# thowell/DirectTrajectoryOptimization.jl

Measured on AMD Instinct MI355X. Metric: SQP iterations/sec + Jacobian nnz/sec, acrobot T=1000, 1->8 GPU, higher is better.
Workload: dtype f64; 1 GPU; acrobot swing-up, implicit midpoint h=0.05, T=1000, exact Hessians, 524288 independent instances per GPU (BASELINE.json configs[2]); horizon=1000, instances_per_gpu=524288, instances_total=524288, num_variables=4999, num_constraint=4004, jacobian_nnz=25982, hessian_key=40971, parallelism=instance sharding x1

## Files before the change

directtrajectoryoptimization.jl_amd/csrc/dto_solver.cpp:

```cpp
#include <hip/hip_runtime.h>

#include <algorithm>
#include <chrono>
#include <cmath>
#include <cstdio>
#include <cstdint>
#include <cstdlib>
#include <cstring>
#include <vector>

#include "../../include/dto.h"
#include "dto_kkt_kernels.hpp"
#include "dto_im_kernels.hpp"
#include "dto_wide_kernels.hpp"
#include "dto_border_kernels.hpp"
#include "dto_problem.hpp"
#include "dto_host_globalization.hpp"

#define HIP_TRY(expr)                                       \
  do {                                                      \
    hipError_t e_ = (expr);                                 \
    if (e_ != hipSuccess) return dto::hip_fail(e_, #expr);  \
  } while (0)

namespace dto {


struct SolverBufs {
  DevBuf<double> wtile;
  DevBuf<int> d_inst_of_slot, d_src_slot;
  DevBuf<double> repack_tmp;
  DevBuf<double> sigx, sigc;
  DevBuf<int> d_ioff;
  DevBuf<int64_t> d_recoff, d_facoff;
  DevBuf<dto_stage_run> d_runs;
  DevBuf<double> d_lo, d_hi;
  DevBuf<double> z, lam, zl, zu, s, zs;
  DevBuf<int> tile_fwd_tag, tile_bwd_tag, fwd_started;
  DevBuf<double> qn;
  DevBuf<double> refq, refvz, refvl, rec_bak;
  DevBuf<double> z_alt, lam_alt;
  DevBuf<double> dz, dlam, ds;
  DevBuf<double> rec, fac, part, lspart, scal, filt;
  DevBuf<double> csum, sfac, xsep, cacc, cpart;
  DevBuf<int> csync;
  DevBuf<int> d_cstart_all;
};

struct SolverState : SolverBufs {
  int64_t B = 0;
  int G = 0;
  int64_t Ni = 0, rec_total = 0, fac_total = 0, n_bnd = 0;
  bool use_wtile = false;
  int G_active = 0;
  std::vector<int> inst_of_slot, slot_of_inst;
  bool use_sigx = false, use_sigc = false, assembled = false;
  std::vector<int> ioff;
  std::vector<int64_t> recoff, facoff;
  int n_runs = 0;
  int sweep_tag = 0;
  hipStream_t stream_lo = nullptr;
  hipEvent_t ev_fork = nullptr, ev_join = nullptr;
  SolverState* cols = nullptr;
  int fuse_state = 0;
  int sb = 8;
  int P = 1;
  int P0 = 1;
  int P_cap = 1;
  int forced_P = 0;
  int n_simd = 1024;
  std::vector<int> cstart;
  int* d_cstart = nullptr;
  dto_kkt_info info{};
  dto_solver_opts opt{};
  dto_options user{};
  bool begun = false;
  std::vector<double> h_scal;

  void release() {
    static_cast<SolverBufs&>(*this) = SolverBufs();
    d_cstart = nullptr; n_runs = 0; fuse_state = 0; sweep_tag = 0;
    if (stream_lo) { (void)hipStreamDestroy(stream_lo); stream_lo = nullptr; }
    if (ev_fork) { (void)hipEventDestroy(ev_fork); ev_fork = nullptr; }
    if (ev_join) { (void)hipEventDestroy(ev_join); ev_join = nullptr; }
    use_wtile = false;
    use_sigx = use_sigc = assembled = false;
    G_active = 0;
    inst_of_slot.clear(); slot_of_inst.clear();
    B = 0; G = 0;
    delete cols; cols = nullptr;
  }
  ~SolverState() { release(); }
};
template <class S>
struct ReleaseOnError {
  S* s;
  ~ReleaseOnError() { if (s) s->release(); }
};

struct ImBufs {
  DevBuf<int> d_aoff, d_doff, d_coff, d_boff, d_ioff;
  DevBuf<double> d_lo, d_hi;
  DevBuf<double> A, R, D, C, Bd;
  DevBuf<double> part, lspart, scal, filt, wbuf;
  DevBuf<int> phase;
  DevBuf<int> lists;
  DevBuf<int> ctr;
};
struct ImState : ImBufs {
  int64_t B = 0;
  dto_im_info info{};
  std::vector<int> aoff, doff, coff, boff, ioff;
  int64_t a_total = 0, d_total = 0, c_total = 0, b_total = 0, Ni = 0, n_bnd = 0;
  bool use_w = false;
  int* h_ctr = nullptr;
  int nwin_e = 1, nwin_l = 1;
  dto_solver_opts opt{};
  dto_options user{};
  bool begun = false;
  int iter_base = 0;
  int64_t passes = 0;
  std::vector<double> h_scal;

  void release() {
    static_cast<ImBufs&>(*this) = ImBufs();
    if (h_ctr) (void)hipHostFree(h_ctr);
    h_ctr = nullptr;
    B = 0; begun = false; use_w = false;
  }
  ~ImState() { release(); }
};

static void default_opts(dto_solver_opts& o, const dto_options& u) {
  o.tol = u.tol; o.s_max = u.s_max; o.dual_inf_tol = u.dual_inf_tol; o.constr_viol_tol = u.constr_viol_tol;
  o.compl_inf_tol = u.compl_inf_tol; o.max_iter = u.max_iter;
  o.acceptable_tol = u.acceptable_tol; o.acceptable_iter = u.acceptable_iter; o.acceptable_dual_inf_tol = u.acceptable_dual_inf_tol;
  o.acceptable_constr_viol_tol = u.acceptable_constr_viol_tol; o.acceptable_compl_inf_tol = u.acceptable_compl_inf_tol;
  o.acceptable_obj_change_tol = u.acceptable_obj_change_tol;
  o.diverging_iterates_tol = u.diverging_iterates_tol; o.mu_target = u.mu_target;
  o.mu_init = u.mu_init; o.kappa_eps = 10.0; o.kappa_mu = 0.2; o.theta_mu = 1.5; o.tau_min = 0.99;
  o.bound_push = 1e-2; o.bound_frac = 1e-2;
  o.delta_c = u.delta_c; o.delta_w_init = u.delta_w_init; o.delta_w_min = 1e-20; o.delta_w_max = 1e20;
  if (const char* e = getenv("DTO_DW_FLOOR")) { const double v = atof(e); if (v > 0.0) o.delta_w_min = v; }
  o.kappa_w_minus = 1.0 / 3.0; o.kappa_w_plus = 8.0; o.kappa_w_plus_first = 100.0;
  o.delta_w_exact_cap = 100.0;
  if (const char* e = getenv("DTO_EXACT_CAP")) o.delta_w_exact_cap = atof(e);
  o.eta_armijo = 1e-4; o.rho_penalty = 0.1; o.piv_tol = 1e-9;
  o.max_refactor = 9;
  o.watchdog_trigger = 2; o.watchdog_trials = 4;
  if (const char* e = getenv("DTO_WATCHDOG")) sscanf(e, "%d,%d", &o.watchdog_trigger, &o.watchdog_trials);
  o.newton_only = 0; o.fixed_delta_w = 0.0;
  o.warm = 0; o.mu_warm = 0.0;
  o.ls_penalty = u.line_search == DTO_LS_PENALTY_FILTER ? 1 : 0; o.ls_switch = u.penalty_switch_theta;
  if (const char* e = getenv("DTO_LS_MERIT")) o.ls_penalty = atoi(e);
  o.pen_gn = 1;
  o.qn_lbfgs = u.hessian_approximation == DTO_HESSIAN_LBFGS ? 1 : 0;
  o.cost_hess_scale = o.qn_lbfgs ? 0.0 : 1.0;
  if (const char* e = getenv("DTO_PEN_GN")) o.pen_gn = atoi(e);
}

struct BorderStats;

static int bordered_step(Problem* p, const dto_batch* b, const double* mu, int64_t ldmu, const double* dw, double delta_c,
                         double* dx, int64_t lddx, double* dmu, int64_t lddmu, int* ok_out, BorderStats* stats, bool pin_fixed = false,
                         const double* gdiag = nullptr, const double* gshift = nullptr);
static int general_solve_batch(Problem* p, const dto_options* opt, const dto_batch* b, double* x_out, int64_t ldxo,
                               double* mu_out, int64_t ldmuo, int32_t* status, int32_t* iterations);

struct WideKkt {
  int64_t B = 0;
  bool assembled = false, factored = false, own_params = false, use_sigx = false, use_sigc = false;
  double delta_w = 0.0, delta_c = 0.0;
  DevBuf<double> z, mu, params, sigx, sigc;
  DevBuf<int> flags;
  DevBuf<double> ws;
  DevBuf<double> ref_r, ref_d;
};
struct KktBorder {
  bool valid = false;
  int nb = 0;
  int64_t B = 0;
  DevBuf<double> g, y;
  DevBuf<double> part;
  DevBuf<double> lu, yw;
  DevBuf<double> v0;
  DevBuf<int> iw;
};
static inline void kkt_border_taken(Problem* p) {
  if (p->kkt_border) p->kkt_border->valid = false;
}
static inline void wide_fac_taken(Problem* p) {
  if (p->wide_kkt) p->wide_kkt->factored = false;
  kkt_border_taken(p);
}
static inline void wide_args_no_linear(dto_wide_args& a) {
  a.sigma_x = a.sigma_c = nullptr; a.ldsx = a.ldsc = 0; a.nneg = nullptr;
  a.rhs_x = a.rhs_c = nullptr; a.ldrx = a.ldrc = 0;
  a.nrhs = a.rhs0 = 0; a.ws = nullptr;
  a.kmul_s = 0;
}

static int wide_step(Problem* p, const dto_batch* b, const double* mu, int64_t ldmu, double delta_w, double delta_c,
                     double* dx, int64_t lddx, double* dmu, int64_t lddmu, int* inertia_ok) {
  int rc = p->ensure_device();
  if (rc) return rc;
  dto_wide_info info;
  p->vt->wide_info(&info);
  const Layout& L = p->L;
  if (L.Nstage != 0 || L.Ngen != 0) return set_error(DTO_ERR_UNSUPPORTED, "wide-stage models: dynamics rows and bounds only");
  hipStream_t st = (hipStream_t)b->stream;
  wide_fac_taken(p);
  const size_t need = (size_t)b->B * (size_t)L.T * (size_t)info.fac_stage;
  HIP_TRY(p->wide_fac.grow(need));
  HIP_TRY(p->wide_flags.grow((size_t)b->B));
  dto_wide_args a;
  a.T = L.T; a.B = b->B;
  a.kind = p->d_kind; a.zoff = p->d_zoff; a.woff = p->d_woff; a.cdoff = p->d_cdoff;
  a.params = b->params ? b->params : p->d_params; a.ldw = b->params ? b->ldp : 0;
  a.z = b->x; a.ldz = b->ldx; a.mu = mu; a.ldmu = ldmu;
  a.delta_w = delta_w; a.delta_c = delta_c; a.piv_tol = 1e-9;
  a.dz = dx; a.lddz = lddx; a.dmu = dmu; a.lddmu = lddmu;
  a.fac = p->wide_fac; a.flags = p->wide_flags; a.Nc = L.Nc;
  a.fixed_lo = a.fixed_hi = nullptr; a.ldb = 0; a.dw_inst = nullptr; a.gam_inst = nullptr; a.active = nullptr; a.stats = nullptr; a.merit = nullptr;
  a.zl = a.zu = nullptr; a.mu_inst = nullptr; a.tau_min = 0.99;
  wide_args_no_linear(a);
  a.prof = nullptr;
  if (const char* e = getenv("DTO_WIDE_PROF")) a.prof = (long long*)(uintptr_t)strtoull(e, nullptr, 0);
  const int lrc = p->vt->launch_wide(DTO_WIDE_STEP, &a, (void*)st);
  if (lrc != 0) return hip_fail((hipError_t)lrc, "wide kernel launch");
  if (inertia_ok) {
    std::vector<int> fl((size_t)b->B);
    HIP_TRY(hipMemcpyAsync(fl.data(), p->wide_flags, fl.size() * sizeof(int), hipMemcpyDeviceToHost, st));
    HIP_TRY(hipStreamSynchronize(st));
    *inertia_ok = 1;
    for (int v : fl) if (!v) *inertia_ok = 0;
  }
  return DTO_OK;
// ... 882 lines not shown
  for (int t = 0; t < L.T; ++t) {
    const int k = L.kind[t];
    S.ioff[t + 1] = S.ioff[t] + S.info.n_ineq[k];
    S.recoff[t + 1] = S.recoff[t] + S.info.rec_size[k];
    S.facoff[t + 1] = S.facoff[t] + (seq_only ? S.info.fac_size_seq[k] : S.info.fac_size[k]);
  }
  S.Ni = S.ioff[L.T]; S.rec_total = S.recoff[L.T]; S.fac_total = S.facoff[L.T];
  for (int64_t rows : {(int64_t)L.Nz, (int64_t)L.Nc, (int64_t)L.Nw, (int64_t)S.Ni, S.rec_total, S.fac_total})
    if (rows >= (int64_t)1 << 22)
      return set_error(DTO_ERR_UNSUPPORTED, "problem too large for the solver path: an array of one instance exceeds 4194303 rows");
  S.n_bnd = S.Ni;
  for (int64_t i = 0; i < L.Nz; ++i) {
    if (L.var_lo[i] == L.var_hi[i]) continue;
    if (std::isfinite(L.var_lo[i])) ++S.n_bnd;
    if (std::isfinite(L.var_hi[i])) ++S.n_bnd;
  }
  {
    std::vector<dto_stage_run> runs;
    auto bounded = [&](int t) {
      for (int i = L.zoff[t]; i < L.zoff[t] + L.nx[t] + L.nu[t]; ++i)
        if (L.var_lo[i] == L.var_hi[i] || std::isfinite(L.var_lo[i]) || std::isfinite(L.var_hi[i])) return 1;
      return 0;
    };
    auto zstep = [&](int t) { return t + 1 < L.T ? L.zoff[t + 1] - L.zoff[t] : L.nx[t] + L.nu[t]; };
    for (int t = 0; t < L.T;) {
      dto_stage_run r{};
      r.kind = L.kind[t]; r.t0 = t; r.bounded = bounded(t);
      r.z0 = L.zoff[t]; r.cd0 = L.cdoff[t]; r.cc0 = L.ccoff[t]; r.io0 = S.ioff[t]; r.w0 = L.woff[t];
      r.rec0 = S.recoff[t]; r.fac0 = S.facoff[t];
      r.zs = zstep(t);
      int e = t + 1;
      if (e < L.T && L.kind[e] == r.kind && bounded(e) == r.bounded && zstep(e) == r.zs && L.zoff[e] - L.zoff[t] == r.zs) {
        r.cds = L.cdoff[e] - L.cdoff[t]; r.ccs = L.ccoff[e] - L.ccoff[t]; r.ios = S.ioff[e] - S.ioff[t]; r.ws = L.woff[e] - L.woff[t];
        r.recs = S.recoff[e] - S.recoff[t]; r.facs = S.facoff[e] - S.facoff[t];
        for (;; ++e) {
          if (e >= L.T || L.kind[e] != r.kind || bounded(e) != r.bounded || zstep(e) != r.zs) break;
          const int64_t n = e - t;
          if (L.zoff[e] != r.z0 + n * r.zs || L.cdoff[e] != r.cd0 + n * r.cds || L.ccoff[e] != r.cc0 + n * r.ccs ||
              S.ioff[e] != r.io0 + n * r.ios || L.woff[e] != r.w0 + n * r.ws || S.recoff[e] != r.rec0 + n * r.recs ||
              S.facoff[e] != r.fac0 + n * r.facs)
            break;
        }
      }
      r.t1 = e;
      runs.push_back(r);
      t = e;
    }
    S.n_runs = (int)runs.size();
    HIP_TRY(S.d_runs.alloc(runs.size()));
    HIP_TRY(hipMemcpy(S.d_runs, runs.data(), runs.size() * sizeof(dto_stage_run), hipMemcpyHostToDevice));
  }
  const size_t lanes = (size_t)S.G * 64;
  HIP_TRY(S.d_ioff.alloc(L.T + 1));
  HIP_TRY(hipMemcpy(S.d_ioff, S.ioff.data(), (L.T + 1) * sizeof(int), hipMemcpyHostToDevice));
  HIP_TRY(S.d_recoff.alloc(L.T + 1));
  HIP_TRY(hipMemcpy(S.d_recoff, S.recoff.data(), (L.T + 1) * sizeof(int64_t), hipMemcpyHostToDevice));
  HIP_TRY(S.d_facoff.alloc(L.T + 1));
  HIP_TRY(hipMemcpy(S.d_facoff, S.facoff.data(), (L.T + 1) * sizeof(int64_t), hipMemcpyHostToDevice));
  HIP_TRY(S.d_lo.alloc(L.Nz));
  HIP_TRY(S.d_hi.alloc(L.Nz));
  HIP_TRY(hipMemcpy(S.d_lo, L.var_lo.data(), L.Nz * sizeof(double), hipMemcpyHostToDevice));
  HIP_TRY(hipMemcpy(S.d_hi, L.var_hi.data(), L.Nz * sizeof(double), hipMemcpyHostToDevice));
  HIP_TRY(S.z.alloc_zeroed(lanes * L.Nz));
  HIP_TRY(S.lam.alloc_zeroed(lanes * L.Nc));
  if (S.n_bnd > S.Ni) {
    HIP_TRY(S.zl.alloc_zeroed(lanes * L.Nz));
    HIP_TRY(S.zu.alloc_zeroed(lanes * L.Nz));
  }
  HIP_TRY(S.s.alloc_zeroed(lanes * S.Ni));
  HIP_TRY(S.zs.alloc_zeroed(lanes * S.Ni));
  HIP_TRY(S.dz.alloc_zeroed(lanes * L.Nz));
  HIP_TRY(S.dlam.alloc_zeroed(lanes * L.Nc));
  HIP_TRY(S.ds.alloc_zeroed(lanes * S.Ni));
  HIP_TRY(S.rec.alloc_zeroed(lanes * S.rec_total));
  HIP_TRY(S.fac.alloc_zeroed(lanes * S.fac_total));
  {
    const int64_t want = ((int64_t)S.G * L.T) / 1024;
    S.sb = (int)std::max<int64_t>(1, std::min<int64_t>(DTO_SB, want));
    if (const char* e = getenv("DTO_STAGE_BLOCK")) S.sb = std::max(1, std::min((int)DTO_SB, atoi(e)));
  }
  const size_t nblk = ((size_t)L.T + S.sb - 1) / S.sb;
  HIP_TRY(S.part.alloc_zeroed(lanes * nblk * S.info.npart));
  HIP_TRY(S.lspart.alloc_zeroed(lanes * nblk * 2 * S.info.ls_trials));
  HIP_TRY(S.scal.alloc_zeroed(lanes * S.info.nscal));
  HIP_TRY(S.tile_fwd_tag.alloc_zeroed((size_t)S.G + 8));
  HIP_TRY(S.tile_bwd_tag.alloc_zeroed((size_t)S.G + 8));
  HIP_TRY(S.fwd_started.alloc_zeroed(16));
  HIP_TRY(S.filt.alloc_zeroed(lanes * 2 * S.info.filter_cap));
  {
    const int q_lo = (S.P_cap > S.P) ? 1 : S.P, q_hi = S.P_cap;
    std::vector<int> all;
    int off_cur = 0;
    for (int q = q_lo; q <= q_hi; ++q) {
      if (q == S.P) off_cur = (int)all.size();
      for (int c = 0; c <= q; ++c) all.push_back((int)(((int64_t)c * L.T) / q));
    }
    S.cstart.assign(all.begin() + off_cur, all.begin() + off_cur + S.P + 1);
    HIP_TRY(S.d_cstart_all.alloc(all.size()));
    HIP_TRY(hipMemcpy(S.d_cstart_all, all.data(), all.size() * sizeof(int), hipMemcpyHostToDevice));
    S.d_cstart = S.d_cstart_all + off_cur;
  }
  HIP_TRY(S.csum.alloc_zeroed(lanes * (size_t)S.P_cap * S.info.chunk_sum_size));
  HIP_TRY(S.sfac.alloc_zeroed(lanes * (size_t)S.P_cap * S.info.sep_fac_size));
  HIP_TRY(S.xsep.alloc_zeroed(lanes * (size_t)S.P_cap * S.info.nx));
  HIP_TRY(S.cacc.alloc_zeroed(lanes * (size_t)S.P_cap * 4));
  HIP_TRY(S.cpart.alloc_zeroed(lanes * (size_t)S.P_cap * 16));
  HIP_TRY(S.csync.alloc_zeroed((size_t)S.G * 4));
  S.h_scal.assign(lanes * S.info.nscal, 0.0);
  HIP_TRY(hipDeviceSynchronize());
  guard.s = nullptr;
  return DTO_OK;
}

static void fill_kkt_args(Problem* p, dto_kkt_args& a) {
  SolverState& S = *p->solver;
  const Layout& L = p->L;
  std::memset(&a, 0, sizeof(a));
  a.T = L.T; a.B = S.B; a.G = S.G;
  a.Nz = L.Nz; a.Nc = L.Nc - L.Ngen; a.Ni = S.Ni;
  a.n_mult = L.Nc; a.n_bnd = S.n_bnd;
  a.kind = p->d_kind; a.zoff = p->d_zoff; a.woff = p->d_woff; a.cdoff = p->d_cdoff; a.ccoff = p->d_ccoff;
  a.ioff = S.d_ioff; a.recoff = S.d_recoff; a.facoff = S.d_facoff;
  a.rec_total = S.rec_total; a.fac_total = S.fac_total;
  a.runs = S.d_runs; a.n_runs = S.n_runs;
  a.lo = S.d_lo; a.hi = S.d_hi; a.params = p->d_params;
  a.wtile = S.use_wtile ? S.wtile : nullptr; a.Nw = L.Nw;
  a.sigx = (S.opt.newton_only && S.use_sigx) ? S.sigx : nullptr;
  a.sigc = (S.opt.newton_only && S.use_sigc) ? S.sigc : nullptr;
  a.z_next = nullptr; a.lam_next = nullptr;
  a.tile_fwd_tag = a.tile_bwd_tag = nullptr; a.sweep_tag = 0; a.fwd_started = nullptr;
  a.z = S.z; a.lam = S.lam; a.zl = S.zl; a.zu = S.zu; a.s = S.s; a.zs = S.zs;
  a.dz = S.dz; a.dlam = S.dlam; a.ds = S.ds;
  a.rec = S.rec; a.fac = S.fac; a.part = S.part; a.lspart = S.lspart; a.scal = S.scal; a.filt = S.filt;
  a.inst_of_slot = S.d_inst_of_slot;
  a.fwd_rounds = fwd_rounds_per_launch();
  a.qn = S.qn; a.qn_mode = 0; a.qn_col = 0;
  a.refq = S.refq; a.refvz = S.refvz; a.refvl = S.refvl;
  a.prof = nullptr;
  if (const char* e = getenv("DTO_KKT_PROF")) a.prof = (long long*)(uintptr_t)strtoull(e, nullptr, 0);
  a.P = S.P; a.cstart = S.d_cstart; a.csum = S.csum; a.sfac = S.sfac; a.xsep = S.xsep; a.cacc = S.cacc; a.cpart = S.cpart;
  a.sb = S.sb;
  {
    const char* e = getenv("DTO_FUSE_JOIN");
    const char* mt = getenv("DTO_FUSE_JOIN_TILES");
    const int max_tiles = mt ? atoi(mt) : 2;
    a.csync = ((!e || atoi(e) != 0) && (S.G_active > 0 ? S.G_active : S.G) <= max_tiles) ? S.csync : nullptr;
  }
  {
    const char* e = getenv("DTO_SEP_CR");
    const bool cr_on = !e || atoi(e) != 0;
    a.sep_cr = !cr_on ? 0 : (S.B <= DTO_SEP_CR_MAX_INST ? 1 : (S.P >= 16 ? 2 : 0));
  }
  a.opt = S.opt;
}

static bool fused_update_available(Problem* p) {
  SolverState& S = *p->solver;
  if (const char* e = getenv("DTO_FUSE_UPDATE")) if (atoi(e) == 0) return false;
  if (S.opt.qn_lbfgs) return false;
  if (S.fuse_state != 0) return S.fuse_state > 0;
  S.fuse_state = -1;
  const size_t lanes = (size_t)S.G * 64;
  const size_t need = lanes * (size_t)(p->L.Nz + p->L.Nc) * sizeof(double);
  size_t free_b = 0, total_b = 0;
  static const double reserve_gb = [] { const char* e = getenv("DTO_FUSE_RESERVE_GB"); return e ? atof(e) : -1.0; }();
  if (hipMemGetInfo(&free_b, &total_b) != hipSuccess) return false;
  const size_t reserve = reserve_gb >= 0.0 ? (size_t)(reserve_gb * 1073741824.0) : total_b / 8;
  if (free_b < need + reserve) return false;
  if (S.z_alt.alloc(lanes * p->L.Nz) != hipSuccess) return false;
  if (S.lam_alt.alloc(lanes * p->L.Nc) != hipSuccess) { S.z_alt.reset(); return false; }
  S.fuse_state = 1;
  return true;
}

static int kkt_launch(Problem* p, int op, const dto_kkt_args& a, hipStream_t st) {
  LaunchTrace* tr = (p->trace && p->trace->on && p->trace->recs.size() < LaunchTrace::MAX_RECS) ? p->trace : nullptr;
  int e0 = -1, e1 = -1;
  if (tr) {
    e0 = tr->take(); e1 = tr->take();
    if (e0 < 0 || e1 < 0) tr = nullptr;
    else HIP_TRY(hipEventRecord(tr->pool[(size_t)e0], st));
  }
  const int rc = p->vt->launch_kkt(op, &a, (void*)st);
  if (rc != 0) return hip_fail((hipError_t)rc, "KKT kernel launch");
  if (tr) {
    HIP_TRY(hipEventRecord(tr->pool[(size_t)e1], st));
    tr->recs.push_back({op, tr->iteration, e0, e1});
  }
  return DTO_OK;
}

static int ensure_refine_buffers(Problem* p, dto_kkt_args& a) {
  SolverState& S = *p->solver;
  const size_t lanes = (size_t)S.G * 64;
  if (!S.refq) HIP_TRY(S.refq.alloc_zeroed(lanes * (size_t)p->L.T * (size_t)S.info.nx));
  if (!S.refvz) HIP_TRY(S.refvz.alloc_zeroed(lanes * (size_t)p->L.Nz));
  if (!S.refvl) HIP_TRY(S.refvl.alloc_zeroed(lanes * (size_t)std::max<int64_t>(1, p->L.Nc)));
  if (!S.rec_bak) HIP_TRY(S.rec_bak.alloc_zeroed(lanes * (size_t)S.rec_total));
  a.refq = S.refq; a.refvz = S.refvz; a.refvl = S.refvl;
  return DTO_OK;
}
template <class F>
static int refine_pass(Problem* p, dto_kkt_args& a, hipStream_t st, F&& solve) {
  SolverState& S = *p->solver;
  int rc;
  const size_t rec_bytes = (size_t)a.G * 64 * (size_t)S.rec_total * sizeof(double);
  HIP_TRY(hipMemcpyAsync(S.rec_bak, S.rec, rec_bytes, hipMemcpyDeviceToDevice, st));
  if ((rc = kkt_launch(p, DTO_KKT_REFINE, a, st))) return rc;
  if ((rc = solve())) return rc;
  HIP_TRY(hipMemcpyAsync(S.rec, S.rec_bak, rec_bytes, hipMemcpyDeviceToDevice, st));
  return kkt_launch(p, DTO_KKT_REFINE_APPLY, a, st);
}

static int pack(Problem* p, dto_kkt_args a, int which, const double* src, int64_t ld, hipStream_t st) {
  a.aos_in = src; a.ld_aos = ld; a.aos_which = which;
  return kkt_launch(p, DTO_KKT_PACK, a, st);
}
static int unpack(Problem* p, dto_kkt_args a, int which, double* dst, int64_t ld, hipStream_t st) {
  a.aos_out = dst; a.ld_aos = ld; a.aos_which = which;
  return kkt_launch(p, DTO_KKT_UNPACK, a, st);
}

static int set_batch_params(Problem* p, const dto_batch* b, hipStream_t st) {
  SolverState& S = *p->solver;
  S.use_wtile = false;
  if (!b->params || p->L.Nw == 0) return DTO_OK;
  if (b->ldp < p->L.Nw) return set_error(DTO_ERR_INVALID, "ldp < num_parameters");
  if (!S.wtile) HIP_TRY(S.wtile.alloc_zeroed((size_t)S.G * 64 * (size_t)p->L.Nw));
  S.use_wtile = true;
  dto_kkt_args a;
  fill_kkt_args(p, a);
  return pack(p, a, 4, b->params, b->ldp, st);
}

static int fetch_scalars(Problem* p, hipStream_t st) {
  SolverState& S = *p->solver;
  HIP_TRY(hipMemcpyAsync(S.h_scal.data(), S.scal, S.h_scal.size() * sizeof(double), hipMemcpyDeviceToHost, st));
  HIP_TRY(hipStreamSynchronize(st));
  return DTO_OK;
}

static inline double hscal(const SolverState& S, int64_t inst, int slot) {
  const int64_t pos = S.slot_of_inst.empty() ? inst : S.slot_of_inst[(size_t)inst];
  return S.h_scal[((pos >> 6) * S.info.nscal + slot) * 64 + (pos & 63)];
}

static void reset_slot_map(SolverState& S) {
  S.d_inst_of_slot.reset();
  S.inst_of_slot.clear(); S.slot_of_inst.clear();
  S.G_active = S.G;
}

static __global__ void k_gather_rows(double* dst, const double* src, int64_t n, const int* src_slot, unsigned nrb) {
  const int64_t tile = blockIdx.x / nrb;
  const int lane = threadIdx.x & 63;
  const int64_t i = (int64_t)(blockIdx.x % nrb) * 4 + (threadIdx.x >> 6);
  if (i >= n) return;
  const int ss = src_slot[tile * 64 + lane];
  dst[((tile * n + i) << 6) + lane] = src[((((int64_t)(ss >> 6)) * n + i) << 6) + (ss & 63)];
}

static __global__ void k_gather_rows_of(double* dst, const double* src, int64_t n, int64_t total, int64_t row0, const int* src_slot,
                                        unsigned nrb) {
  const int64_t tile = blockIdx.x / nrb;
  const int lane = threadIdx.x & 63;
  const int64_t i = (int64_t)(blockIdx.x % nrb) * 4 + (threadIdx.x >> 6);
  if (i >= n) return;
  const int ss = src_slot[tile * 64 + lane];
  dst[((tile * n + i) << 6) + lane] = src[((((int64_t)(ss >> 6)) * total + row0 + i) << 6) + (ss & 63)];
}

static int repack(Problem* p, hipStream_t st, int* n_running_out) {
  SolverState& S = *p->solver;
  const Layout& L = p->L;
  const int lanes = S.G * 64;
  if (S.info.quasi_newton) { if (n_running_out) *n_running_out = -1; return DTO_OK; }
  if (S.inst_of_slot.empty()) {
    S.inst_of_slot.resize(lanes); S.slot_of_inst.resize(lanes);
    for (int i = 0; i < lanes; ++i) S.inst_of_slot[i] = S.slot_of_inst[i] = i;
  }
  std::vector<int> src(lanes);
  int nrun = 0, k = 0;
  auto running = [&](int slot) {
    return S.inst_of_slot[slot] < S.B && S.h_scal[(((size_t)slot >> 6) * S.info.nscal + SC_STATUS) * 64 + (slot & 63)] == 0.0;
  };
  for (int sl = 0; sl < lanes; ++sl) if (running(sl)) src[k++] = sl;
  nrun = k;
  for (int sl = 0; sl < lanes; ++sl) if (!running(sl)) src[k++] = sl;
  if (n_running_out) *n_running_out = nrun;
  const int g_new = std::max(1, (nrun + 63) / 64);
  if (g_new >= S.G_active) return DTO_OK;
  if (!S.d_src_slot) HIP_TRY(S.d_src_slot.alloc(lanes));
  if (!S.d_inst_of_slot) HIP_TRY(S.d_inst_of_slot.alloc(lanes));
  HIP_TRY(hipMemcpyAsync(S.d_src_slot, src.data(), lanes * sizeof(int), hipMemcpyHostToDevice, st));
  int64_t widest = std::max<int64_t>(std::max<int64_t>(L.Nz, L.Nc), std::max<int64_t>(S.info.nscal, L.Nw));
  widest = std::max<int64_t>(widest, std::max<int64_t>(S.Ni, 2 * (int64_t)S.info.filter_cap));
  const size_t need = (size_t)lanes * (size_t)widest;
  HIP_TRY(S.repack_tmp.grow(need));
  auto move = [&](double* buf, int64_t n) -> int {
    if (!buf || n <= 0) return DTO_OK;
    const unsigned nrb = (unsigned)((n + 3) / 4);
    if ((uint64_t)nrb * (uint64_t)S.G > 0x7fffffffull) return set_error(DTO_ERR_INVALID, "batch too large to repack");
    hipLaunchKernelGGL(k_gather_rows, dim3(nrb * (unsigned)S.G), dim3(256), 0, st, S.repack_tmp, (const double*)buf, n,
                       (const int*)S.d_src_slot, nrb);
    HIP_TRY(hipGetLastError());
    HIP_TRY(hipMemcpyAsync(buf, S.repack_tmp, (size_t)lanes * (size_t)n * sizeof(double), hipMemcpyDeviceToDevice, st));
// ... 988 lines not shown
    const size_t live = (size_t)std::min<int64_t>(64, S.B - (int64_t)g * 64);
    HIP_TRY(hipMemsetAsync(S.scal + ((size_t)g * S.info.nscal + SC_STATUS) * 64, 0, live * sizeof(double), st));
  }
  if ((rc = dto::kkt_launch(p, DTO_KKT_FACTOR_SOLVE, a, st))) return rc;
  if ((rc = dto::unpack(p, a, 2, dx, lddx, st))) return rc;
  if ((rc = dto::unpack(p, a, 3, dmu, lddmu, st))) return rc;
  if (inertia_ok) {
    if ((rc = dto::fetch_scalars(p, st))) return rc;
    *inertia_ok = 1;
    for (int64_t i = 0; i < S.B; ++i)
      if (dto::hscal(S, i, SC_LS_FAIL) != 0.0) *inertia_ok = 0;
  }
  S.begun = false;
  return DTO_OK;
}

namespace dto {
static __global__ __launch_bounds__(64) void k_qn_cols_copy(dto_kkt_args am, dto_kkt_args ac, int ncol, int nblk) {
  const int64_t gc = blockIdx.x / nblk;
  const int blk = blockIdx.x % nblk;
  const int lc = threadIdx.x;
  const int64_t sc_ = gc * 64 + lc, ms = sc_ / ncol;
  const int64_t gm = ms >> 6;
  const int lm = (int)(ms & 63);
  const bool in_range = gm < am.G;
  auto rows = [&](double* dst, const double* src, int64_t n) {
    if (!dst || !src || n == 0 || !in_range) return;
    const int64_t r0 = (n * blk) / nblk, r1 = (n * (blk + 1)) / nblk;
    for (int64_t r = r0; r < r1; ++r) dst[((gc * n + r) << 6) + lc] = src[((gm * n + r) << 6) + lm];
  };
  rows(ac.z, am.z, am.Nz);
  rows(ac.lam, am.lam, am.Nc);
  rows(ac.zl, am.zl, am.Nz);
  rows(ac.zu, am.zu, am.Nz);
  rows(ac.s, am.s, am.Ni);
  rows(ac.zs, am.zs, am.Ni);
  if (am.wtile && ac.wtile) rows(const_cast<double*>(ac.wtile), am.wtile, am.Nw);
  if (in_range) {
    const int64_t n = am.rec_total, r0 = (n * blk) / nblk, r1 = (n * (blk + 1)) / nblk;
    for (int64_t r = r0; r < r1; ++r)
      ac.rec[((gc * n) << 6) + ((r >> 1) << 7) + 2 * lc + (r & 1)] = am.rec[((gm * n) << 6) + ((r >> 1) << 7) + 2 * lm + (r & 1)];
  }
  if (blk == 0) {
    for (int k = 0; k < SC_COUNT; ++k)
      ac.scal[((gc * SC_COUNT + k) << 6) + lc] = in_range ? am.scal[((gm * SC_COUNT + k) << 6) + lm] : (k == SC_STATUS ? DTO_ST_NO_INSTANCE : 0.0);
  }
}
static __global__ __launch_bounds__(64) void k_qn_cols_gather(dto_kkt_args am, dto_kkt_args ac, int ncol, int nblk) {
  const int64_t gm = blockIdx.x / ((int64_t)ncol * nblk);
  const int rem = (int)(blockIdx.x % ((int64_t)ncol * nblk));
  const int c = rem / nblk, blk = rem % nblk;
  const int lm = threadIdx.x;
  if (am.scal[((gm * SC_COUNT + SC_STATUS) << 6) + lm] != 0.0) return;
  const int64_t sc_ = (gm * 64 + lm) * ncol + c, gc = sc_ >> 6;
  const int lc = (int)(sc_ & 63);
  const QnRows R{am.Nz};
  double* q = am.qn + ((gm * R.total()) << 6) + lm;
  const int64_t n = am.Nz, r0 = (n * blk) / nblk, r1 = (n * (blk + 1)) / nblk;
  for (int64_t r = r0; r < r1; ++r) q[(R.Z(c) + r) << 6] = ac.dz[((gc * n + r) << 6) + lc] - q[(R.v0() + r) << 6];
}
}

int dto_solver_begin(dto_problem* h, const dto_options* opt, const dto_batch* b) {
  Problem* p = reinterpret_cast<Problem*>(h);
  if (!p || !b || !b->x) return set_error(DTO_ERR_INVALID, "null argument");
  if (b->ldx < p->L.Nz) return set_error(DTO_ERR_INVALID, "ldx < num_variables");
  if (p->vt->launch_wide) return dto::wide_begin(p, opt, b, false, 0.0);
  int rc = p->ensure_device();
  if (rc) return rc;
  if (p->solver) p->solver->begun = false;
  if (p->im) p->im->begun = false;
  p->im_active = false;
  if (dto::use_im(p, b->B)) {
    if ((rc = dto::ensure_im_state(p, b->B))) return rc;
    if ((rc = dto::im_begin(p, opt, b, false, 0.0))) return rc;
    p->im_active = true;
    p->hessian_mode_last = DTO_HESSIAN_EXACT;
    return DTO_OK;
  }
  rc = dto::ensure_state(p, b->B);
  if (rc) return rc;
  SolverState& S = *p->solver;
  dto::reset_slot_map(S);
  S.use_sigx = S.use_sigc = S.assembled = false;
  if ((rc = dto::set_batch_params(p, b, (hipStream_t)b->stream))) return rc;
  dto_options u;
  if (opt) u = *opt; else dto_options_default(&u);
  S.user = u;
  dto::default_opts(S.opt, u);
  if (S.info.quasi_newton) S.opt.pen_gn = 0;
  hipStream_t st = (hipStream_t)b->stream;
  if (S.opt.qn_lbfgs && S.info.quasi_newton) S.opt.qn_lbfgs = 0;
  p->hessian_mode_last = S.info.quasi_newton ? DTO_HESSIAN_SR1_BLOCKS : (S.opt.qn_lbfgs ? DTO_HESSIAN_LBFGS : DTO_HESSIAN_EXACT);
  if (S.opt.qn_lbfgs) {
    if (p->L.Ngen != 0)
      return set_error(DTO_ERR_UNSUPPORTED, "hessian_approximation = limited-memory: lane-per-instance solver path without GeneralConstraint rows");
    const size_t need = (size_t)S.G * (size_t)dto::QnRows{p->L.Nz}.total() * 64;
    HIP_TRY(S.qn.grow(need));
    HIP_TRY(hipMemsetAsync(S.qn, 0, need * sizeof(double), st));
    const char* ce = getenv("DTO_QN_COLS");
    const bool cols_on = !ce || atoi(ce) != 0;
    if (cols_on && (int64_t)S.G * 64 * dto::QN_M2 <= 65536) {
      if (!S.cols) S.cols = new dto::SolverState();
      dto::SolverState& C = *S.cols;
      C.forced_P = 0;
      p->solver = &C;
      rc = dto::ensure_state(p, (int64_t)S.G * 64 * dto::QN_M2);
      p->solver = &S;
      if (rc) return rc;
      C.opt = S.opt; C.user = S.user;
      dto::reset_slot_map(C);
      C.use_sigx = C.use_sigc = C.assembled = false;
      C.use_wtile = false;
      if (S.use_wtile) {
        if (!C.wtile) HIP_TRY(C.wtile.alloc_zeroed((size_t)C.G * 64 * (size_t)p->L.Nw));
        C.use_wtile = true;
      }
    } else if (S.cols) {
      delete S.cols; S.cols = nullptr;
    }
  }
  dto_kkt_args a;
  dto::fill_kkt_args(p, a);
  const size_t lanes = (size_t)S.G * 64;
  if (S.csync) HIP_TRY(hipMemsetAsync(S.csync, 0, (size_t)S.G * 4 * sizeof(int), st));
  HIP_TRY(hipMemsetAsync(S.lam, 0, std::max<size_t>(1, lanes * p->L.Nc) * sizeof(double), st));
  if ((rc = dto::pack(p, a, 0, b->x, b->ldx, st))) return rc;
  if ((rc = dto::kkt_launch(p, DTO_KKT_INIT, a, st))) return rc;
  S.begun = true;
  (void)dto::fused_update_available(p);
  return DTO_OK;
}

int dto_solver_iterate(dto_problem* h, int n, void* stream) {
  Problem* p = reinterpret_cast<Problem*>(h);
  if (p && p->im_active && p->im && p->im->begun) return dto::im_iterate(p, n, (hipStream_t)stream);
  if (p && p->vt->launch_wide) {
    if (!p->wide || !p->wide->begun) return set_error(DTO_ERR_INVALID, "dto_solver_begin has not been called");
    return dto::wide_iterate(p, std::max(0, n), (hipStream_t)stream);
  }
  if (!p || !p->solver || !p->solver->begun) return set_error(DTO_ERR_INVALID, "dto_solver_begin has not been called");
  hipStream_t st = (hipStream_t)stream;
  dto_kkt_args a;
  dto::fill_kkt_args(p, a);
  if (p->solver->G_active > 0) a.G = p->solver->G_active;
  int rc;
  SolverState& S = *p->solver;
  const int n_fused = dto::fused_update_available(p) ? ((n - 1) / 2) * 2 : 0;
  const bool qn = S.opt.qn_lbfgs != 0;
  const bool overlap = !qn && dto::overlap_sweeps(p, st);
  static const bool gate = [] { const char* e = getenv("DTO_OVERLAP_GATE"); return !e || atoi(e) != 0; }();
  const int n_refine = (!qn && !S.info.quasi_newton && S.user.kkt_refinement > 0) ? std::min(S.user.kkt_refinement, 4) : 0;
  if (n_refine > 0 && (rc = dto::ensure_refine_buffers(p, a))) return rc;
  for (int it = 0; it < n; ++it) {
    if (p->trace && p->trace->on && it > 0) ++p->trace->iteration;
    if (it > 0 && it <= n_fused) {
      a.z_next = S.z_alt; a.lam_next = S.lam_alt;
      if ((rc = dto::kkt_launch(p, DTO_KKT_UPDATE_EVAL, a, st))) return rc;
      std::swap(S.z, S.z_alt); std::swap(S.lam, S.lam_alt);
      a.z = S.z; a.lam = S.lam; a.z_next = nullptr; a.lam_next = nullptr;
    } else {
      if ((rc = dto::kkt_launch(p, DTO_KKT_EVAL, a, st))) return rc;
    }
    if (qn && (rc = dto::kkt_launch(p, DTO_KKT_QN_BEGIN, a, st))) return rc;
    if ((rc = dto::kkt_launch(p, DTO_KKT_CONV, a, st))) return rc;
    auto factor_solve = [&]() -> int {
    if (overlap) {
      a.tile_fwd_tag = S.tile_fwd_tag; a.tile_bwd_tag = S.tile_bwd_tag; a.sweep_tag = ++S.sweep_tag;
      a.fwd_started = gate ? S.fwd_started : nullptr;
      if (gate) HIP_TRY(hipMemsetAsync(S.fwd_started, 0, sizeof(int), st));
      HIP_TRY(hipEventRecord(S.ev_fork, st));
      HIP_TRY(hipStreamWaitEvent(S.stream_lo, S.ev_fork, 0));
      if ((rc = dto::kkt_launch(p, DTO_KKT_FWD, a, st))) return rc;
      if (gate && (rc = dto::kkt_launch(p, DTO_KKT_BWD_GATE, a, S.stream_lo))) return rc;
      {
        static const int passes = [] { const char* e = getenv("DTO_OVERLAP_PASSES"); return e ? atoi(e) : 1; }();
        for (int k = 0; k < passes; ++k)
          if ((rc = dto::kkt_launch(p, DTO_KKT_BWD_EARLY, a, S.stream_lo))) return rc;
      }
      HIP_TRY(hipEventRecord(S.ev_join, S.stream_lo));
      HIP_TRY(hipStreamWaitEvent(st, S.ev_join, 0));
      if ((rc = dto::kkt_launch(p, DTO_KKT_BWD_REST, a, st))) return rc;
      if ((rc = dto::kkt_launch(p, DTO_KKT_POST, a, st))) return rc;
      a.tile_fwd_tag = a.tile_bwd_tag = nullptr; a.fwd_started = nullptr;
    } else {
      if ((rc = dto::kkt_launch(p, DTO_KKT_FACTOR_SOLVE, a, st))) return rc;
    }
    return DTO_OK;
    };
    if ((rc = factor_solve())) return rc;
    for (int r = 0; r < n_refine; ++r)
      if ((rc = dto::refine_pass(p, a, st, factor_solve))) return rc;
    if (qn) {
      a.qn_col = -1;
      if ((rc = dto::kkt_launch(p, DTO_KKT_QN_COL, a, st))) return rc;
      if (S.cols) {
        dto::SolverState& C = *S.cols;
        dto_kkt_args ac;
        p->solver = &C;
        dto::fill_kkt_args(p, ac);
        p->solver = &S;
        ac.qn_main = S.qn;
        ac.opt = a.opt;
        const int nblk = 16;
        hipLaunchKernelGGL(dto::k_qn_cols_copy, dim3((unsigned)((int64_t)C.G * nblk)), dim3(64), 0, st, a, ac, (int)dto::QN_M2, nblk);
        HIP_TRY(hipGetLastError());
        if ((rc = dto::kkt_launch(p, DTO_KKT_QN_COLS_RHS, ac, st))) return rc;
        if ((rc = dto::kkt_launch(p, DTO_KKT_FACTOR_SOLVE, ac, st))) return rc;
        hipLaunchKernelGGL(dto::k_qn_cols_gather, dim3((unsigned)((int64_t)a.G * dto::QN_M2 * nblk)), dim3(64), 0, st, a, ac, (int)dto::QN_M2, nblk);
        HIP_TRY(hipGetLastError());
      } else {
        for (int col = 0; col < dto::QN_M2; ++col) {
          a.qn_mode = 0; a.qn_col = col;
          if ((rc = dto::kkt_launch(p, DTO_KKT_QN_RHS, a, st))) return rc;
          if ((rc = dto::kkt_launch(p, DTO_KKT_FACTOR_SOLVE, a, st))) return rc;
          if ((rc = dto::kkt_launch(p, DTO_KKT_QN_COL, a, st))) return rc;
        }
      }
      if ((rc = dto::kkt_launch(p, DTO_KKT_QN_SMALL, a, st))) return rc;
      a.qn_mode = 1;
      if ((rc = dto::kkt_launch(p, DTO_KKT_QN_RHS, a, st))) return rc;
      if ((rc = dto::kkt_launch(p, DTO_KKT_FACTOR_SOLVE, a, st))) return rc;
      a.qn_mode = 2;
      if ((rc = dto::kkt_launch(p, DTO_KKT_QN_RHS, a, st))) return rc;
      a.qn_mode = 0; a.qn_col = 0;
    }
    if ((rc = dto::kkt_launch(p, DTO_KKT_LINESEARCH, a, st))) return rc;
    if ((rc = dto::kkt_launch(p, DTO_KKT_LS_REDUCE, a, st))) return rc;
    if (qn && (rc = dto::kkt_launch(p, DTO_KKT_QN_SAVE, a, st))) return rc;
    if (!(it + 1 < n && it + 1 <= n_fused))
      if ((rc = dto::kkt_launch(p, DTO_KKT_UPDATE, a, st))) return rc;
  }
  if (p->trace && p->trace->on) ++p->trace->iteration;
  return DTO_OK;
}

int dto_solver_hessian_mode(dto_problem* h, int* mode) {
  Problem* p = reinterpret_cast<Problem*>(h);
  if (!p || !mode) return set_error(DTO_ERR_INVALID, "null argument");
  *mode = p->hessian_mode_last;
  return DTO_OK;
}

int dto_solver_trace(dto_problem* h, int on) {
  Problem* p = reinterpret_cast<Problem*>(h);
  if (!p) return set_error(DTO_ERR_INVALID, "null argument");
  if (p->vt->launch_wide) return set_error(DTO_ERR_UNSUPPORTED, "dto_solver_trace: the tile path has no launch trace");
  if (!p->trace) p->trace = new dto::LaunchTrace();
  if (on) p->trace->clear();
  p->trace->on = on != 0;
  return DTO_OK;
}

int dto_solver_trace_read(dto_problem* h, int32_t* op, int32_t* iteration, double* start_ms, double* duration_ms, int64_t capacity,
                          int64_t* count) {
  Problem* p = reinterpret_cast<Problem*>(h);
  if (!p || !count) return set_error(DTO_ERR_INVALID, "null argument");
  *count = 0;
  if (!p->trace) return DTO_OK;
  dto::LaunchTrace& T = *p->trace;
  *count = (int64_t)T.recs.size();
  if (T.recs.empty() || capacity <= 0) return DTO_OK;
  HIP_TRY(hipDeviceSynchronize());
  const hipEvent_t origin = T.pool[(size_t)T.recs[0].e0];
  const int64_t n = std::min<int64_t>(capacity, (int64_t)T.recs.size());
  for (int64_t i = 0; i < n; ++i) {
    const dto::LaunchTrace::Rec& r = T.recs[(size_t)i];
    float t0 = 0.f, dt = 0.f;
    HIP_TRY(hipEventElapsedTime(&t0, origin, T.pool[(size_t)r.e0]));
    HIP_TRY(hipEventElapsedTime(&dt, T.pool[(size_t)r.e0], T.pool[(size_t)r.e1]));
    if (op) op[i] = r.op;
    if (iteration) iteration[i] = r.iteration;
    if (start_ms) start_ms[i] = (double)t0;
    if (duration_ms) duration_ms[i] = (double)dt;
  }
  return DTO_OK;
}

int dto_solver_stats(dto_problem* h, int32_t* status, int32_t* iterations, double* objective, double* constr_viol,
                     double* dual_inf, double* mu, double* delta_w, double* alpha) {
  Problem* p = reinterpret_cast<Problem*>(h);
  if (p && p->im_active && p->im && p->im->A) {
    ImState& I = *p->im;
    HIP_TRY(hipDeviceSynchronize());
    int rc = dto::im_fetch_scalars(p, p->stream);
    if (rc) return rc;
    for (int64_t i = 0; i < I.B; ++i) {
      if (status) status[i] = (int32_t)dto::im_hscal(I, i, SC_STATUS);
      if (iterations) iterations[i] = (int32_t)dto::im_hscal(I, i, SC_ITER);
      if (objective) objective[i] = dto::im_hscal(I, i, SC_F);
      if (constr_viol) constr_viol[i] = dto::im_hscal(I, i, SC_THETA_INF);
      if (dual_inf) dual_inf[i] = dto::im_hscal(I, i, SC_DINF);
      if (mu) mu[i] = dto::im_hscal(I, i, SC_MU);
      if (delta_w) delta_w[i] = dto::im_hscal(I, i, SC_DELTA_W);
      if (alpha) alpha[i] = dto::im_hscal(I, i, SC_ALPHA);
    }
    return DTO_OK;
  }
  if (p && p->vt->launch_wide) {
    if (!p->wide || p->wide->I.empty()) return set_error(DTO_ERR_INVALID, "no solver state");
    const dto::WideState& W = *p->wide;
    for (int64_t i = 0; i < W.B; ++i) {
      const dto::WideInst& s = W.I[(size_t)i];
      if (status) status[i] = s.status;
      if (iterations) iterations[i] = s.iter;
      if (objective) objective[i] = s.f;
      if (constr_viol) constr_viol[i] = s.thinf;
      if (dual_inf) dual_inf[i] = s.dinf;
      if (mu) mu[i] = s.mu;
      if (delta_w) delta_w[i] = s.dw;
      if (alpha) alpha[i] = s.alpha;
    }
    return DTO_OK;
  }
  if (!p || !p->solver || !p->solver->z) return set_error(DTO_ERR_INVALID, "no solver state");
  SolverState& S = *p->solver;
  HIP_TRY(hipDeviceSynchronize());
  int rc = dto::fetch_scalars(p, p->stream);
  if (rc) return rc;
  for (int64_t i = 0; i < S.B; ++i) {
    if (status) status[i] = (int32_t)dto::hscal(S, i, SC_STATUS);
    if (iterations) iterations[i] = (int32_t)dto::hscal(S, i, SC_ITER);
    if (objective) objective[i] = dto::hscal(S, i, SC_F);
    if (constr_viol) constr_viol[i] = dto::hscal(S, i, SC_THETA_INF);
    if (dual_inf) dual_inf[i] = dto::hscal(S, i, SC_DINF);
    if (mu) mu[i] = dto::hscal(S, i, SC_MU);
    if (delta_w) delta_w[i] = dto::hscal(S, i, SC_DELTA_W);
    if (alpha) alpha[i] = dto::hscal(S, i, SC_ALPHA);
  }
  return DTO_OK;
}

int dto_solver_launch_op(dto_problem* h, int op, void* stream) {
  Problem* p = reinterpret_cast<Problem*>(h);
  if (p && p->im_active && p->im && p->im->begun) {
    ImState& I = *p->im;
    const int iop = op - 100;
    if (iop < DTO_IM_EVAL || iop > DTO_IM_UPDATE) return set_error(DTO_ERR_INVALID, "op out of range (instance-major engine: 100 + dto_im_op)");
    dto_im_args a;
    dto::fill_im_args(p, a);
    const int k = (iop == DTO_IM_EVAL || iop == DTO_IM_CONV) ? 0 : (iop == DTO_IM_FWD ? 1 : 2);
    a.list = I.lists + (size_t)k * I.B; a.count = I.ctr + k;
    a.ticket = I.ctr + (iop == DTO_IM_BWD ? 4 : 3);
    HIP_TRY(hipMemsetAsync(I.ctr + 3, 0, 2 * sizeof(int), (hipStream_t)stream));
    return dto::im_launch(p, iop, a, (hipStream_t)stream);
  }
  if (p && p->vt->launch_wide) return set_error(DTO_ERR_UNSUPPORTED, "dto_solver_launch_op: the tile path has no per-kernel iteration ops");
  if (!p || !p->solver || !p->solver->begun) return set_error(DTO_ERR_INVALID, "dto_solver_begin has not been called");
  if (op < DTO_KKT_EVAL || op >= DTO_KKT_OP_COUNT) return set_error(DTO_ERR_INVALID, "op out of range");
  dto_kkt_args a;
  dto::fill_kkt_args(p, a);
  if (p->solver->G_active > 0) a.G = p->solver->G_active;
  if (op == DTO_KKT_UPDATE_EVAL) {
    SolverState& S = *p->solver;
    if (!dto::fused_update_available(p)) return set_error(DTO_ERR_UNSUPPORTED, "the fused UPDATE+EVAL pass is not available (memory, DTO_FUSE_UPDATE=0)");
    a.z_next = S.z_alt; a.lam_next = S.lam_alt;
    const int rc = dto::kkt_launch(p, op, a, (hipStream_t)stream);
    if (rc) return rc;
    std::swap(S.z, S.z_alt); std::swap(S.lam, S.lam_alt);
    return DTO_OK;
  }
  if (op == DTO_KKT_REFINE) {
    SolverState& S = *p->solver;
    if (S.info.quasi_newton || S.opt.qn_lbfgs) return set_error(DTO_ERR_UNSUPPORTED, "iterative refinement: exact-Hessian plugins, not in limited-memory mode");
    int rc = dto::ensure_refine_buffers(p, a);
    if (rc) return rc;
    hipStream_t st = (hipStream_t)stream;
    return dto::refine_pass(p, a, st, [&]() { return dto::kkt_launch(p, DTO_KKT_FACTOR_SOLVE, a, st); });
  }
  if (op == DTO_KKT_REFINE_APPLY) return set_error(DTO_ERR_INVALID, "DTO_KKT_REFINE_APPLY is part of DTO_KKT_REFINE");
  return dto::kkt_launch(p, op, a, (hipStream_t)stream);
}

int dto_solver_set_partitions(dto_problem* h, int partitions) {
  Problem* p = reinterpret_cast<Problem*>(h);
  if (!p || partitions < 0 || partitions > 64) return set_error(DTO_ERR_INVALID, "partitions must be in [0, 64]");
  if (p->vt->launch_wide) return set_error(DTO_ERR_UNSUPPORTED, "dto_solver_set_partitions: the tile path factorises every instance in one workgroup");
  if (partitions > p->L.T) return set_error(DTO_ERR_INVALID, "more partitions than stages");
  if (!p->solver) p->solver = new SolverState();
  p->solver->forced_P = partitions;
  return DTO_OK;
}

static __global__ void k_shift_knots(const double* in, double* out, int64_t ld, int T_blocks, int stride, int last_len, int k) {
  const int64_t b = blockIdx.y;
// ... 694 lines not shown
```

Measured before the change: 2.937 million SQP iterations/s.

## Split instance tiles into two groups on separate streams to overlap sweeps

The solver's tiles are split into two halves, each driven on its own stream (plus an optional low-priority stream per half), with per-group views of all state buffers. Each group runs its own SQP iteration pipeline, and events serialize the forward sweeps across groups so one group's forward sweep can overlap the other's backward sweep, line search and update. The aim is to fill GPU idle gaps from the serial kernel chain and launch bubbles. In exchange it adds event and stream overhead, doubles kernel launches, and makes the two groups compete for CUs.

```diff
diff --git a/directtrajectoryoptimization.jl_amd/csrc/dto_solver.cpp b/directtrajectoryoptimization.jl_amd/csrc/dto_solver.cpp
--- a/directtrajectoryoptimization.jl_amd/csrc/dto_solver.cpp
+++ b/directtrajectoryoptimization.jl_amd/csrc/dto_solver.cpp
@@ -61,6 +61,10 @@
   int sweep_tag = 0;
   hipStream_t stream_lo = nullptr;
   hipEvent_t ev_fork = nullptr, ev_join = nullptr;
+  hipStream_t stream_b = nullptr, stream_b_lo = nullptr;
+  hipEvent_t ev_call_fork = nullptr, ev_call_join = nullptr, ev_fork_b = nullptr, ev_join_b = nullptr;
+  hipEvent_t ev_fwd[4] = {nullptr, nullptr, nullptr, nullptr};
+  bool stream_b_lo_failed = false;
   SolverState* cols = nullptr;
   int fuse_state = 0;
   int sb = 8;
@@ -83,6 +87,11 @@
     if (stream_lo) { (void)hipStreamDestroy(stream_lo); stream_lo = nullptr; }
     if (ev_fork) { (void)hipEventDestroy(ev_fork); ev_fork = nullptr; }
     if (ev_join) { (void)hipEventDestroy(ev_join); ev_join = nullptr; }
+    for (hipStream_t* s : {&stream_b, &stream_b_lo})
+      if (*s) { (void)hipStreamDestroy(*s); *s = nullptr; }
+    for (hipEvent_t* e : {&ev_call_fork, &ev_call_join, &ev_fork_b, &ev_join_b, &ev_fwd[0], &ev_fwd[1], &ev_fwd[2], &ev_fwd[3]})
+      if (*e) { (void)hipEventDestroy(*e); *e = nullptr; }
+    stream_b_lo_failed = false;
     use_wtile = false;
     use_sigx = use_sigc = assembled = false;
     G_active = 0;
@@ -1271,6 +1280,56 @@
     a.sep_cr = !cr_on ? 0 : (S.B <= DTO_SEP_CR_MAX_INST ? 1 : (S.P >= 16 ? 2 : 0));
   }
   a.opt = S.opt;
+}
+
+static dto_kkt_args group_view(const SolverState& S, const dto_kkt_args& a, int g0, int n) {
+  dto_kkt_args v = a;
+  const int64_t lane0 = (int64_t)g0 << 6;
+  auto adv = [&](auto*& ptr, int64_t rows) { if (ptr) ptr += lane0 * rows; };
+  v.G = n;
+  if (a.inst_of_slot) v.inst_of_slot = a.inst_of_slot + lane0;
+  else v.B = std::max<int64_t>(0, std::min<int64_t>((int64_t)n << 6, a.B - lane0));
+  adv(v.z, a.Nz); adv(v.lam, a.Nc); adv(v.zl, a.Nz); adv(v.zu, a.Nz); adv(v.s, a.Ni); adv(v.zs, a.Ni);
+  adv(v.z_next, a.Nz); adv(v.lam_next, a.Nc);
+  adv(v.dz, a.Nz); adv(v.dlam, a.Nc); adv(v.ds, a.Ni);
+  adv(v.rec, a.rec_total); adv(v.fac, a.fac_total);
+  const int64_t nblk = ((int64_t)a.T + a.sb - 1) / a.sb;
+  adv(v.part, nblk * S.info.npart); adv(v.lspart, nblk * 2 * S.info.ls_trials);
+  adv(v.scal, S.info.nscal); adv(v.filt, 2 * (int64_t)S.info.filter_cap);
+  adv(v.csum, (int64_t)a.P * S.info.chunk_sum_size); adv(v.sfac, (int64_t)a.P * S.info.sep_fac_size);
+  adv(v.xsep, (int64_t)a.P * S.info.nx); adv(v.cacc, (int64_t)a.P * 4); adv(v.cpart, (int64_t)a.P * 16);
+  if (v.csync) v.csync += (int64_t)g0 * 4;
+  adv(v.wtile, a.Nw); adv(v.sigx, a.Nz); adv(v.sigc, a.Nc);
+  if (v.tile_fwd_tag) v.tile_fwd_tag += g0;
+  if (v.tile_bwd_tag) v.tile_bwd_tag += g0;
+  return v;
+}
+
+static int tile_groups(Problem* p, hipStream_t st) {
+  SolverState& S = *p->solver;
+  const int tiles = S.G_active > 0 ? S.G_active : S.G;
+  int want = 2;
+  if (const char* e = getenv("DTO_TILE_GROUPS")) want = atoi(e);
+  if (want != 2 || tiles < 2) return 1;
+  if (S.P != 1 || S.opt.qn_lbfgs || S.info.quasi_newton || S.user.kkt_refinement > 0 || S.opt.newton_only) return 1;
+  if (fwd_rounds_per_launch() > 0) return 1;
+  hipStreamCaptureStatus cs = hipStreamCaptureStatusNone;
+  if (st && hipStreamIsCapturing(st, &cs) == hipSuccess && cs != hipStreamCaptureStatusNone) return 1;
+  if (!S.stream_b && hipStreamCreateWithFlags(&S.stream_b, hipStreamNonBlocking) != hipSuccess) { S.stream_b = nullptr; return 1; }
+  for (hipEvent_t* e : {&S.ev_call_fork, &S.ev_call_join, &S.ev_fork_b, &S.ev_join_b, &S.ev_fwd[0], &S.ev_fwd[1], &S.ev_fwd[2], &S.ev_fwd[3]})
+    if (!*e && hipEventCreateWithFlags(e, hipEventDisableTiming) != hipSuccess) { *e = nullptr; return 1; }
+  return 2;
+}
+static bool group_b_lo_stream(SolverState& S) {
+  if (S.stream_b_lo) return true;
+  if (S.stream_b_lo_failed) return false;
+  int lo = 0, hi = 0;
+  if (hipDeviceGetStreamPriorityRange(&lo, &hi) != hipSuccess ||
+      hipStreamCreateWithPriority(&S.stream_b_lo, hipStreamNonBlocking, lo) != hipSuccess) {
+    S.stream_b_lo = nullptr; S.stream_b_lo_failed = true;
+    return false;
+  }
+  return true;
 }
 
 static bool fused_update_available(Problem* p) {
@@ -2565,45 +2624,58 @@
   static const bool gate = [] { const char* e = getenv("DTO_OVERLAP_GATE"); return !e || atoi(e) != 0; }();
   const int n_refine = (!qn && !S.info.quasi_newton && S.user.kkt_refinement > 0) ? std::min(S.user.kkt_refinement, 4) : 0;
   if (n_refine > 0 && (rc = dto::ensure_refine_buffers(p, a))) return rc;
-  for (int it = 0; it < n; ++it) {
-    if (p->trace && p->trace->on && it > 0) ++p->trace->iteration;
-    if (it > 0 && it <= n_fused) {
-      a.z_next = S.z_alt; a.lam_next = S.lam_alt;
-      if ((rc = dto::kkt_launch(p, DTO_KKT_UPDATE_EVAL, a, st))) return rc;
-      std::swap(S.z, S.z_alt); std::swap(S.lam, S.lam_alt);
-      a.z = S.z; a.lam = S.lam; a.z_next = nullptr; a.lam_next = nullptr;
-    } else {
-      if ((rc = dto::kkt_launch(p, DTO_KKT_EVAL, a, st))) return rc;
-    }
-    if (qn && (rc = dto::kkt_launch(p, DTO_KKT_QN_BEGIN, a, st))) return rc;
-    if ((rc = dto::kkt_launch(p, DTO_KKT_CONV, a, st))) return rc;
-    auto factor_solve = [&]() -> int {
-    if (overlap) {
-      a.tile_fwd_tag = S.tile_fwd_tag; a.tile_bwd_tag = S.tile_bwd_tag; a.sweep_tag = ++S.sweep_tag;
-      a.fwd_started = gate ? S.fwd_started : nullptr;
-      if (gate) HIP_TRY(hipMemsetAsync(S.fwd_started, 0, sizeof(int), st));
-      HIP_TRY(hipEventRecord(S.ev_fork, st));
-      HIP_TRY(hipStreamWaitEvent(S.stream_lo, S.ev_fork, 0));
-      if ((rc = dto::kkt_launch(p, DTO_KKT_FWD, a, st))) return rc;
-      if (gate && (rc = dto::kkt_launch(p, DTO_KKT_BWD_GATE, a, S.stream_lo))) return rc;
+  struct Group { int g0, n; hipStream_t st, lo; hipEvent_t fork, join; int* started; };
+  const int ng = dto::tile_groups(p, st);
+  const int n_a = ng == 2 ? (a.G + 1) / 2 : a.G;
+  Group grp[2] = {{0, n_a, st, overlap ? S.stream_lo : nullptr, S.ev_fork, S.ev_join, S.fwd_started},
+                  {n_a, a.G - n_a, S.stream_b, nullptr, S.ev_fork_b, S.ev_join_b, S.fwd_started + 1}};
+  if (ng == 2 && overlap && dto::group_b_lo_stream(S)) grp[1].lo = S.stream_b_lo;
+  const bool one_fwd_at_a_time = a.G > S.n_simd;
+  hipEvent_t last_fwd = nullptr;
+  int n_fwd = 0;
+  auto factor_solve =[&](dto_kkt_args& v, const Group& g) -> int {
+    if (ng == 1 && !g.lo) return dto::kkt_launch(p, DTO_KKT_FACTOR_SOLVE, v, g.st);
+    if (ng == 2 && last_fwd && (one_fwd_at_a_time || n_fwd == 1)) HIP_TRY(hipStreamWaitEvent(g.st, last_fwd, 0));
+    if (g.g0 == 0) ++S.sweep_tag;
+    if (g.lo) {
+      v.tile_fwd_tag = S.tile_fwd_tag + g.g0; v.tile_bwd_tag = S.tile_bwd_tag + g.g0; v.sweep_tag = S.sweep_tag;
+      v.fwd_started = gate ? g.started : nullptr;
+      if (gate) HIP_TRY(hipMemsetAsync(g.started, 0, sizeof(int), g.st));
+      HIP_TRY(hipEventRecord(g.fork, g.st));
+      HIP_TRY(hipStreamWaitEvent(g.lo, g.fork, 0));
+    }
+    if ((rc = dto::kkt_launch(p, DTO_KKT_FWD, v, g.st))) return rc;
+    if (ng == 2 && (one_fwd_at_a_time || n_fwd == 0)) {
+      last_fwd = S.ev_fwd[n_fwd & 3];
+      HIP_TRY(hipEventRecord(last_fwd, g.st));
+    }
+    ++n_fwd;
+    if (g.lo) {
+      if (gate && (rc = dto::kkt_launch(p, DTO_KKT_BWD_GATE, v, g.lo))) return rc;
       {
         static const int passes = [] { const char* e = getenv("DTO_OVERLAP_PASSES"); return e ? atoi(e) : 1; }();
         for (int k = 0; k < passes; ++k)
-          if ((rc = dto::kkt_launch(p, DTO_KKT_BWD_EARLY, a, S.stream_lo))) return rc;
+          if ((rc = dto::kkt_launch(p, DTO_KKT_BWD_EARLY, v, g.lo))) return rc;
       }
-      HIP_TRY(hipEventRecord(S.ev_join, S.stream_lo));
-      HIP_TRY(hipStreamWaitEvent(st, S.ev_join, 0));
-      if ((rc = dto::kkt_launch(p, DTO_KKT_BWD_REST, a, st))) return rc;
-      if ((rc = dto::kkt_launch(p, DTO_KKT_POST, a, st))) return rc;
-      a.tile_fwd_tag = a.tile_bwd_tag = nullptr; a.fwd_started = nullptr;
+      HIP_TRY(hipEventRecord(g.join, g.lo));
+      HIP_TRY(hipStreamWaitEvent(g.st, g.join, 0));
+      if ((rc = dto::kkt_launch(p, DTO_KKT_BWD_REST, v, g.st))) return rc;
+      if ((rc = dto::kkt_launch(p, DTO_KKT_POST, v, g.st))) return rc;
+      v.tile_fwd_tag = v.tile_bwd_tag = nullptr; v.fwd_started = nullptr;
     } else {
-      if ((rc = dto::kkt_launch(p, DTO_KKT_FACTOR_SOLVE, a, st))) return rc;
+      if ((rc = dto::kkt_launch(p, DTO_KKT_BWD, v, g.st))) return rc;
+      if ((rc = dto::kkt_launch(p, DTO_KKT_POST, v, g.st))) return rc;
     }
     return DTO_OK;
-    };
-    if ((rc = factor_solve())) return rc;
+  };
+  auto iterate_group = [&](dto_kkt_args& a, const Group& g, int it) -> int {
+    hipStream_t st = g.st;
+    auto factor_solve_here = [&]() -> int { return factor_solve(a, g); };
+    if (qn && (rc = dto::kkt_launch(p, DTO_KKT_QN_BEGIN, a, st))) return rc;
+    if ((rc = dto::kkt_launch(p, DTO_KKT_CONV, a, st))) return rc;
+    if ((rc = factor_solve_here())) return rc;
     for (int r = 0; r < n_refine; ++r)
-      if ((rc = dto::refine_pass(p, a, st, factor_solve))) return rc;
+      if ((rc = dto::refine_pass(p, a, st, factor_solve_here))) return rc;
     if (qn) {
       a.qn_col = -1;
       if ((rc = dto::kkt_launch(p, DTO_KKT_QN_COL, a, st))) return rc;
@@ -2643,7 +2715,48 @@
     if (qn && (rc = dto::kkt_launch(p, DTO_KKT_QN_SAVE, a, st))) return rc;
     if (!(it + 1 < n && it + 1 <= n_fused))
       if ((rc = dto::kkt_launch(p, DTO_KKT_UPDATE, a, st))) return rc;
-  }
+    return DTO_OK;
+  };
+  auto run = [&]() -> int {
+    for (int it = 0; it < n; ++it) {
+      if (p->trace && p->trace->on && it > 0) ++p->trace->iteration;
+      const bool fused = it > 0 && it <= n_fused;
+      if (fused) { a.z_next = S.z_alt; a.lam_next = S.lam_alt; }
+      for (int k = 0; k < ng; ++k) {
+        const dto_kkt_args v = ng == 1 ? a : dto::group_view(S, a, grp[k].g0, grp[k].n);
+        if ((rc = dto::kkt_launch(p, fused ? DTO_KKT_UPDATE_EVAL : DTO_KKT_EVAL, v, grp[k].st))) return rc;
+      }
+      if (fused) {
+        std::swap(S.z, S.z_alt); std::swap(S.lam, S.lam_alt);
+        a.z = S.z; a.lam = S.lam; a.z_next = nullptr; a.lam_next = nullptr;
+      }
+      if (ng == 1) {
+        if ((rc = iterate_group(a, grp[0], it))) return rc;
+      } else {
+        for (int k = 0; k < ng; ++k) {
+          dto_kkt_args v = dto::group_view(S, a, grp[k].g0, grp[k].n);
+          if ((rc = iterate_group(v, grp[k], it))) return rc;
+        }
+      }
+    }
+    return DTO_OK;
+  };
+  if (ng == 2) {
+    HIP_TRY(hipEventRecord(S.ev_call_fork, st));
+    HIP_TRY(hipStreamWaitEvent(S.stream_b, S.ev_call_fork, 0));
+  }
+  rc = run();
+  if (ng == 2) {
+    if (rc) {
+      for (const Group& g : grp)
+        if (g.lo && hipEventRecord(g.join, g.lo) == hipSuccess) (void)hipStreamWaitEvent(g.st, g.join, 0);
+      if (hipEventRecord(S.ev_call_join, S.stream_b) == hipSuccess) (void)hipStreamWaitEvent(st, S.ev_call_join, 0);
+      return rc;
+    }
+    HIP_TRY(hipEventRecord(S.ev_call_join, S.stream_b));
+    HIP_TRY(hipStreamWaitEvent(st, S.ev_call_join, 0));
+  }
+  if (rc) return rc;
   if (p->trace && p->trace->on) ++p->trace->iteration;
   return DTO_OK;
 }
```

New measurement: 2.963 million SQP iterations/s (median of 4 runs). No clear change (+0.9%).
